# mathcom/G2Vec

Hardware: AMD Instinct MI355X
Metric: cbow_paths_per_sec (higher is better)
Workload: dtype fp32; 1 GPU; model=g2vec-cbow, global_batch=60057, seq_len=80, parallelism=dp1, hidden=128, num_repetition=10, num_repetition_global=10, hipgraph_active=True, grad_allreduce_bytes_per_epoch=30092, step_includes=full-batch fwd+bwd+allreduce+dense-Adam + post-update train/val ACC evals

## Files before the change

g2vec_amd/models/cbow.py:

```python
from __future__ import annotations

import dataclasses
import operator
import time
from typing import Any, List, Optional

import torch

from .. import ops
from ..config import G2VecConfig
from ..parallel.dist import DistContext, single
from ..paths import PathSet, subset


class _CpuEvent:
    def record(self):
        pass

    def synchronize(self):
        pass


@dataclasses.dataclass
class TrainResult:
    W_ih: torch.Tensor
    stop_epoch: int
    acc_val: float
    acc_tr: float
    epochs_run: int
    acc_val_history: List[float]
    epoch_times_s: List[float]
    wall_to_acc_s: Optional[float]


@dataclasses.dataclass
class TrainState:
    W: torch.Tensor
    who: torch.Tensor
    mW: torch.Tensor
    vW: torch.Tensor
    mO: torch.Tensor
    vO: torch.Tensor
    W_keep: torch.Tensor
    tr: PathSet
    vl: PathSet
    plan: Any
    inv_b: float
    batches: list
    W16: Optional[torch.Tensor] = None
    t_adam: int = 0
    epoch_idx: int = 0
    s_buf: Optional[torch.Tensor] = None
    lrt_buf: Optional[torch.Tensor] = None
    counts_buf: Optional[torch.Tensor] = None
    dO_buf: Optional[torch.Tensor] = None
    ev_genes: Optional[torch.Tensor] = None
    ev_offsets: Optional[torch.Tensor] = None
    ev_labels: Optional[torch.Tensor] = None
    graph: Any = None
    graph_failed: bool = False
    kbufs: Optional[tuple] = None
    kgraph: Any = None
    kblock_k: Optional[int] = None
    kgraph_failed: bool = False
    run_bufs: Optional[tuple] = None
    pipe_bufs: Optional[tuple] = None


EPOCH_TENSORS = ("W", "who", "mW", "vW", "mO", "vO", "dO_buf")
_epoch_tensors = operator.attrgetter(*EPOCH_TENSORS)


def accuracies(counts, n_tr: int, n_vl: int) -> tuple:
    return float(counts[0]) / max(n_tr, 1), float(counts[1]) / max(n_vl, 1)


def capture_graph(body, log, label: str):
    try:
        g = torch.cuda.CUDAGraph()
        with torch.cuda.graph(g, capture_error_mode="thread_local"):
            body()
        return g
    except Exception as e:
        log(label % repr(e))
        return None


class StopTracker:

    def __init__(self, early_stop: bool, before_val: float = -1.0,
                 before_tr: float = -1.0, hist: Optional[list] = None):
        self.early_stop = early_stop
        self.before_val, self.before_tr = before_val, before_tr
        self.hist: List[float] = hist if hist is not None else []
# ... 159 lines not shown

        use_general = cfg.trainer_path == "general"
        if cfg.batch_size == 0:
            tr = self._locality_sort(tr)
            vl = self._locality_sort(vl)
        plan = ops.build_scatter_plan(tr.genes, tr.offsets, self.G,
                                      slabs=not use_general)
        if self.n_tr_global + self.n_vl_global == 0:
            raise ValueError(
                "no paths to train on: the integrated path set is empty "
                "(every walk was dropped as a cross-group duplicate, or "
                "the PCC-thresholded graphs have no edges — check the "
                "expression signal / --pcc-threshold)")
        P_loc = tr.n_paths
        bs = cfg.batch_size if cfg.batch_size > 0 else max(P_loc, 1)
        st = TrainState(
            W=W, who=who, mW=torch.zeros_like(W), vW=torch.zeros_like(W),
            mO=torch.zeros_like(who), vO=torch.zeros_like(who),
            W_keep=W.clone(), tr=tr, vl=vl, plan=plan,
            inv_b=1.0 / max(self.n_tr_global, 1),
            batches=[(i, min(i + bs, P_loc)) for i in range(0, P_loc, bs)])
        if use_general and cfg.dtype != "fp32":
            st.W16 = (W.bfloat16() if cfg.dtype == "bf16" else W.half())
        if self.ctx.world > 1 and cfg.batch_size > 0:
            nb = torch.tensor([float(len(st.batches))], dtype=torch.float64,
                              device=self.device)
            self.ctx.allreduce_max_(nb)
            while len(st.batches) < int(nb.item()):
                st.batches.append((P_loc, P_loc))
        if not use_general:
            st.s_buf = torch.empty(self.G, dtype=torch.float32,
                                   device=self.device)
            ops.gemv_rows(W, who, st.s_buf)
        st.lrt_buf = torch.zeros(1, dtype=torch.float32, device=self.device)
        st.counts_buf = torch.zeros(2, dtype=torch.float32, device=self.device)
        if not use_general and tr.n_paths + vl.n_paths > 0:
            off_vl = vl.offsets.int() + tr.offsets[-1]
            st.ev_genes = torch.cat([tr.genes, vl.genes]).contiguous()
            st.ev_offsets = torch.cat([tr.offsets, off_vl[1:]]).contiguous()
            st.ev_labels = torch.cat([tr.labels, vl.labels]).contiguous()
        if not use_general and cfg.batch_size == 0:
            st.dO_buf = torch.zeros(tr.n_paths, dtype=torch.float32,
                                    device=self.device)
            if tr.n_paths > 0:
                _l, _c, d0 = ops.cbow_fwd_scalar(
                    st.s_buf, tr.genes, tr.offsets, tr.labels, st.inv_b, True)
                st.dO_buf.copy_(d0)
        return st

    def _epoch_body_fast(self, st, counts_out=None, lrt_slot=None,
                         reduce_counts: bool = True) -> None:
        cfg = self.cfg
        tr, vl = st.tr, st.vl
        if counts_out is None:
            counts_out = st.counts_buf
        if self.device.type != "cuda" or st.ev_genes is None:
            counts_out.zero_()
        if lrt_slot is not None:
            lrt = lrt_slot
        else:
            lrt = st.lrt_buf if self.device.type == "cuda" else None
        c = ops.scatter_dO(tr.genes, tr.offsets, st.dO_buf, self.G,
                           plan=st.plan)
        self.ctx.allreduce_(c)
        ops.adam_rank1_fused(st.W, st.mW, st.vW, c, st.who, st.mO, st.vO,
                             st.t_adam, cfg.lr, self.B1, self.B2, self.EPS,
                             lrt_buf=lrt)
        ops.gemv_rows(st.W, st.who, st.s_buf)
        if st.ev_genes is not None:
            ops.cbow_eval_counts_(st.s_buf, st.ev_genes, st.ev_offsets,
                                  st.ev_labels, tr.n_paths, counts_out,
                                  dO=st.dO_buf, inv_b=st.inv_b)
        if reduce_counts:
            self.ctx.allreduce_(counts_out)

    def run_epoch(self, st) -> tuple:
        cfg = self.cfg
        fast_full = cfg.trainer_path != "general" and cfg.batch_size == 0
        if fast_full:
            self._step_epoch(st)
            return self._accs(st.counts_buf.cpu().numpy())

        for (lo, hi) in st.batches:
            b_inv = (st.inv_b if cfg.batch_size == 0 else
                     (1.0 / ((hi - lo) * self.ctx.world) if hi > lo else 0.0))
            st.t_adam += 1
            if cfg.trainer_path == "general":
                self._step_general(st, lo, hi, b_inv, st.t_adam)
            else:
                self._step_fast(st, lo, hi, b_inv, st.t_adam)
        if cfg.trainer_path == "general":
            acc_tr = self._accuracy(st.W, st.W16, st.who, st.tr, self.n_tr_global)
            acc_val = self._accuracy(st.W, st.W16, st.who, st.vl, self.n_vl_global)
        else:
            ops.gemv_rows(st.W, st.who, st.s_buf)
            counts = torch.empty(2, dtype=torch.float32, device=self.device)
            for k, split in enumerate((st.tr, st.vl)):
                if split.n_paths == 0:
                    counts[k] = 0.0
                    continue
                _l, corr, _d = ops.cbow_fwd_scalar(
                    st.s_buf, split.genes, split.offsets, split.labels, 1.0, False)
                counts[k] = corr.sum()
            self.ctx.allreduce_(counts)
            acc_tr, acc_val = self._accs(counts.cpu().numpy())
# ... 26 lines not shown
                "    (hipGraph capture unavailable: %s; running eager)")
            st.graph_failed = st.graph is None

    def _launch_epoch(self, st, slot: int, pinned, snaps, events,
                      keep: bool = True) -> None:
        self._step_epoch(st)
        pinned[slot].copy_(st.counts_buf, non_blocking=True)
        if keep:
            snaps[slot][0].copy_(st.W)
            snaps[slot][1].copy_(st.who)
        events[slot].record()

    KBLOCK = 8

    def pick_kblock(self, n_epochs: int) -> int:
        n = max(int(n_epochs), 1)
        if n <= 64:
            return n
        for k in range(64, 1, -1):
            if n % k == 0:
                return k
        return self.KBLOCK

    def _ensure_kgraph(self, st, k: Optional[int] = None) -> None:
        if self.device.type != "cuda" or not self.cfg.use_hipgraph:
            return
        if not self.ctx.graph_capture_ok():
            return
        K = max(int(k), 1) if k is not None else (st.kblock_k or self.KBLOCK)
        if st.kbufs is None or st.kbufs[0].numel() != K:
            st.kbufs = (
                torch.empty(K, dtype=torch.float32, device=self.device),
                torch.zeros(K, 2, dtype=torch.float32, device=self.device))
            st.kgraph = None
        if st.kgraph is None and not st.kgraph_failed:
            klrt, kcounts = st.kbufs

            def bodies():
                for j in range(K):
                    self._epoch_body_fast(st, counts_out=kcounts[j],
                                          lrt_slot=klrt[j:j + 1],
                                          reduce_counts=False)
            st.kgraph = capture_graph(
                bodies, self.log, "    (k-epoch block graph unavailable: "
                                  "%s; running per-epoch)")
            if st.kgraph is not None:
                st.kblock_k = K
            else:
                st.kgraph_failed = True

    def kblock_eligible(self, st, n_epochs: int, early_stop: bool) -> bool:
        return (not early_stop and not st.kgraph_failed and
                st.ev_genes is not None and n_epochs >= 2)

    def _run_epochs_kblocked(self, st, n_epochs: int, on_epoch):
        on_gpu = self.device.type == "cuda"
        if st.epoch_idx == 0:
            warm = [self.run_epoch(st)]
        else:
            warm = []
        self._ensure_kgraph(st)
        n_rest = n_epochs - len(warm)
        K = st.kblock_k if st.kgraph is not None else None
        n_blocked = (n_rest // K) * K if K else 0
        sched_vals = torch.tensor(
            [ops.tf1_lr_t(self.cfg.lr, self.B1, self.B2, st.t_adam + i)
             for i in range(1, n_rest + 1)], dtype=torch.float32)
        if on_gpu:
            cap = max(n_rest, 1)
            if st.run_bufs is None or st.run_bufs[0].numel() < cap:
                st.run_bufs = (
                    torch.empty(cap, dtype=torch.float32, pin_memory=True),
                    torch.empty(cap, dtype=torch.float32,
                                device=self.device),
                    torch.zeros(cap, 2, dtype=torch.float32,
# ... 285 lines not shown
```

g2vec_amd/ops/__init__.py:

```python
from __future__ import annotations

from typing import NamedTuple, Optional

import torch

from . import cpu_ref

_NATIVE = None
_NATIVE_ERR: Optional[BaseException] = None
try:
    from g2vec_amd import _C as _NATIVE
except Exception as e:
    _NATIVE_ERR = e


def native_available() -> bool:
    return _NATIVE is not None


def native():
    if _NATIVE is None:
        raise RuntimeError(
            "g2vec_amd._C HIP extension is not importable on this host — the GPU "
            "compute path refuses to fall back to eager PyTorch. Build it in-tree "
            "with `python setup.py build_ext --inplace` (PYTORCH_ROCM_ARCH=gfx950). "
            f"Import error was: {_NATIVE_ERR!r}")
    return _NATIVE


def random_walks(row_ptr, col_idx, weights, sources, num_repetition: int,
                 len_path: int, seed: int):
    if row_ptr.is_cuda:
        return native().random_walks(row_ptr, col_idx, weights, sources,
                                     num_repetition, len_path, seed)
    return cpu_ref.random_walks(row_ptr, col_idx, weights, sources,
                                num_repetition, len_path, seed)


def cbow_fwd_scalar(s, genes, offsets, labels, inv_b: float, want_grad: bool):
    if s.is_cuda:
        loss, correct, dO = native().cbow_fwd_scalar(
            s, genes, offsets, labels, float(inv_b), bool(want_grad))
        return loss, correct, (dO if want_grad else None)
    return cpu_ref.cbow_fwd_scalar(s, genes, offsets, labels, inv_b, want_grad)


def cbow_eval_counts_(s, genes, offsets, labels, p_split: int,
                      counts: torch.Tensor, dO: Optional[torch.Tensor] = None,
                      inv_b: float = 1.0, scan=None) -> None:
    if s.is_cuda:
        if scan is not None:
            pathid, piece, cap = scan
            native().cbow_eval_scan_(s, genes, pathid, offsets, labels,
                                     int(p_split), int(cap), piece, counts,
                                     dO=dO, inv_b=float(inv_b))
            return
        native().cbow_eval_counts_(s, genes, offsets, labels, int(p_split),
                                   counts, dO=dO, inv_b=float(inv_b))
        return
    _l, corr, d = cpu_ref.cbow_fwd_scalar(s, genes, offsets, labels, inv_b,
                                          dO is not None)
    counts[0] += corr[:p_split].sum()
    counts[1] += corr[p_split:].sum()
    if dO is not None:
        dO.copy_(d[:p_split])


class ScatterPlan(NamedTuple):
    inst_path: torch.Tensor
    seg_start: torch.Tensor
    seg_gene: torch.Tensor
    slab_seg_ptr: Optional[list] = None


SLAB_BYTES = 3 << 20


def build_scatter_plan(genes: torch.Tensor, offsets: torch.Tensor,
                       n_genes: int, _force_slabs: bool = False,
                       slabs: bool = True) -> ScatterPlan:
    counts = (offsets[1:] - offsets[:-1]).long()
    P = len(counts)
    path_of = torch.repeat_interleave(
        torch.arange(P, device=genes.device), counts)
    slab_paths = SLAB_BYTES // 4
    n_slabs = ((P + slab_paths - 1) // slab_paths
               if slabs and (genes.is_cuda or _force_slabs) else 1)
    if n_slabs <= 1:
        sorted_key, perm = torch.sort(genes.long(), stable=True)
    else:
        key = (path_of // slab_paths) * n_genes + genes.long()
        sorted_key, perm = torch.sort(key, stable=True)
    inst_path = path_of[perm].int().contiguous()
    seg_key, seg_counts = torch.unique_consecutive(sorted_key,
                                                   return_counts=True)
    seg_start = torch.zeros(len(seg_key) + 1, dtype=torch.int64,
                            device=genes.device)
    torch.cumsum(seg_counts, 0, out=seg_start[1:])
    if n_slabs <= 1:
        return ScatterPlan(inst_path, seg_start.int().contiguous(),
                           seg_key.int().contiguous())
    seg_slab = seg_key // n_genes
    seg_gene = (seg_key - seg_slab * n_genes).int().contiguous()
    ptr = torch.searchsorted(
        seg_slab, torch.arange(n_slabs + 1, device=genes.device)).cpu()
    return ScatterPlan(inst_path, seg_start.int().contiguous(), seg_gene,
                       [int(x) for x in ptr])


def _plan_slabs(plan: ScatterPlan):
    ptr = plan.slab_seg_ptr
    if ptr is None:
        if plan.seg_gene.numel():
            yield plan.seg_start, plan.seg_gene
        return
    for a, b in zip(ptr[:-1], ptr[1:]):
        if b > a:
            yield plan.seg_start[a:b + 1], plan.seg_gene[a:b]


def scatter_dO(genes, offsets, dO, n_genes: int,
               plan: Optional[ScatterPlan] = None):
    if dO.is_cuda:
        if plan is None:
            plan = build_scatter_plan(genes, offsets, n_genes)
        c = torch.zeros(n_genes, dtype=torch.float32, device=dO.device)
        for seg_start, seg_gene in _plan_slabs(plan):
            native().scatter_dO_det_(plan.inst_path, seg_start, seg_gene,
                                     dO, c)
        return c
    return cpu_ref.scatter_dO(genes, offsets, dO, n_genes)


def trunc_normal_(out: torch.Tensor, std: float, seed: int) -> None:
    if out.is_cuda:
        native().trunc_normal_(out, float(std), int(seed))
        return
    cpu_ref.trunc_normal_(out, std, seed)


def tf1_lr_t(lr: float, b1: float, b2: float, t: int) -> float:
    return lr * (1.0 - b2 ** t) ** 0.5 / (1.0 - b1 ** t)


def _lrt_buf(lrt_buf, W, t: int, lr: float, b1: float, b2: float):
    if lrt_buf is not None:
        return lrt_buf
    return torch.tensor([tf1_lr_t(lr, b1, b2, t)], dtype=torch.float32,
                        device=W.device)


def adam_rank1(W, m, v, c, who, t: int, lr: float, b1: float, b2: float,
               eps: float, lrt_buf: Optional[torch.Tensor] = None) -> None:
    if W.is_cuda:
        lrt_buf = _lrt_buf(lrt_buf, W, t, lr, b1, b2)
        native().adam_rank1(W, m, v, c, who, lrt_buf, float(b1), float(b2),
                            float(eps))
        return
    cpu_ref.adam_rank1(W, m, v, c, who, t, lr, b1, b2, eps)


def adam_rank1_fused(W, m, v, c, who, mO, vO, t: int, lr: float,
                     b1: float, b2: float, eps: float,
# ... 18 lines not shown
    cpu_ref.adam_dense(W, m, v, grad, t, lr, b1, b2, eps)


def cbow_fwd(W, who, genes, offsets, labels, inv_b: float, want_grad: bool,
             act: int = 0):
    if W.is_cuda:
        loss, correct, dO, H = native().cbow_fwd(
            W, who, genes, offsets, labels, float(inv_b), bool(want_grad),
            act=int(act))
        if not want_grad:
            return loss, correct, None, None
        return loss, correct, dO, H
    return cpu_ref.cbow_fwd(W, who, genes, offsets, labels, inv_b, want_grad,
                            act=act)


def cbow_bwd_rows(who, genes, offsets, dO, n_genes: int,
                  plan: Optional[ScatterPlan] = None,
                  H_pre: Optional[torch.Tensor] = None):
    if dO.is_cuda:
        if plan is None:
            plan = build_scatter_plan(genes, offsets, n_genes, slabs=False)
        if plan.slab_seg_ptr is not None:
            raise RuntimeError(
                "cbow_bwd_rows needs a single-pass plan "
                "(build_scatter_plan(..., slabs=False)), got a slab-blocked one")
        return native().cbow_bwd_rows(who, plan.inst_path, plan.seg_start,
                                      plan.seg_gene, dO, int(n_genes),
                                      Hpre=H_pre)
    return cpu_ref.cbow_bwd_rows(who, genes, offsets, dO, n_genes,
                                 H_pre=H_pre)


def gemv_rows(W, x, out) -> None:
    if W.is_cuda:
        native().gemv_rows_(W, x, out)
        return
    torch.mv(W, x, out=out)


def gemv_cols(W, c, out) -> None:
    if W.is_cuda:
        native().gemv_cols_(W, c, out)
        return
    torch.mv(W.t(), c, out=out)


REP_MAX = 32


def _rep_R(t: torch.Tensor, name: str) -> int:
    if t.dim() != 2 or t.dtype != torch.float32 or not t.is_contiguous():
        raise ValueError(f"{name} must be a contiguous float32 [rows, R] tensor")
    R = int(t.shape[1])
    if not 1 <= R <= REP_MAX:
        raise ValueError(f"{name}: R must be in [1, {REP_MAX}], got {R}")
    return R


def cbow_eval_counts_rep_(s_R, genes, offsets, labels, p_split: int,
                          counts_R: torch.Tensor,
                          dO_R: Optional[torch.Tensor] = None,
                          inv_b: float = 1.0) -> None:
    R = _rep_R(s_R, "s_R")
    if s_R.is_cuda:
        native().cbow_eval_counts_rep_(s_R, genes, offsets, labels,
                                       int(p_split), counts_R, dO_R=dO_R,
                                       inv_b=float(inv_b))
        return
    for r in range(R):
        cnt = torch.zeros(2, dtype=torch.float32)
# ... 270 lines not shown
```

g2vec_amd/ops/csrc/bindings.hip:

```cpp
#include <torch/extension.h>
#include <c10/hip/HIPStream.h>
#include <hip/hip_runtime.h>

#include <climits>
#include <cstdio>
#include <functional>
#include <initializer_list>
#include <optional>
#include <cstring>
#include <fstream>
#include <sstream>
#include <string>
#include <type_traits>
#include <vector>

#include "g2vec_kernels.hip"

namespace {

inline void check_gpu_cont(const torch::Tensor& t, const char* name) {
  TORCH_CHECK(t.is_cuda(), name, " must be on the GPU");
  TORCH_CHECK(t.is_contiguous(), name, " must be contiguous");
}
inline void check_f32(const torch::Tensor& t, const char* name) {
// ... 157 lines not shown
inline void check_offs(const torch::Tensor& offs, long long P) {
  TORCH_CHECK(offs.numel() == P + 1, "offs must have P + 1 elements");
}
inline void check_p_split(long long p_split, long long P) {
  TORCH_CHECK(p_split >= 0 && p_split <= P, "p_split must be in [0, P]");
}
inline void check_seg_start(const torch::Tensor& seg_start, int n_seg) {
  TORCH_CHECK(seg_start.numel() == (long long)n_seg + 1,
              "seg_start must have n_seg + 1 elements");
}

std::vector<torch::Tensor> cbow_fwd_scalar(torch::Tensor s, torch::Tensor genes,
                                           torch::Tensor offs, torch::Tensor labels,
                                           double inv_b, bool want_grad) {
  CHECK_F32(s); CHECK_I32(genes); CHECK_I32(offs); CHECK_F32(labels);
  check_same_device(s, {genes, offs, labels});
  const long long P = labels.numel();
  check_offs(offs, P);
  auto loss = torch::empty({P}, opts_on(s));
  auto correct = torch::empty({P}, opts_on(s));
  auto dO = torch::empty({want_grad ? P : 0}, opts_on(s));
  if (P == 0) return {loss, correct, dO};
  launch(cbow_fwd_scalar_kernel, grid_for(P, 16, 2048), 0, f32(s), i32(genes),
         i32(offs), f32(labels), P, inv_b, f32(loss), f32(correct),
         want_grad ? f32(dO) : nullptr);
  return {loss, correct, dO};
}

void fold_partials(const torch::Tensor& partials, torch::Tensor& counts) {
  launch(fold_partials_kernel, 1, 0, f32(partials), partials.size(0),
         f32(counts));
}

void cbow_eval_counts_(torch::Tensor s, torch::Tensor genes, torch::Tensor offs,
                       torch::Tensor labels, int64_t p_split,
                       torch::Tensor counts,
                       std::optional<torch::Tensor> dO, double inv_b) {
  if (dO) {
    CHECK_F32(*dO);
    TORCH_CHECK(dO->numel() >= p_split,
                "dO must cover the train split (p < p_split)");
  }
  CHECK_F32(s); CHECK_I32(genes); CHECK_I32(offs); CHECK_F32(labels);
  CHECK_F32(counts);
  check_same_device(s, {genes, offs, labels, counts});
  if (dO) check_same_device(s, {*dO});
  TORCH_CHECK(counts.numel() == 2, "counts must have 2 elements");
  const long long P = labels.numel();
  check_offs(offs, P);
  check_p_split(p_split, P);
  if (P == 0) return;
  const long long G = s.numel();
  const char* lds_env = getenv("G2VEC_EVAL_LDS");
  const long long lds_cap = lds_env ? atoll(lds_env) : 0;
  const bool lds = G * 4 <= lds_cap && G * 4 <= 158 * 1024;
  const int grid =
      grid_for(P, 16, lds ? env_int_min1("G2VEC_EVAL_LDS_GRID", 1024)
                          : env_int_min1("G2VEC_EVAL_GRID", 2048));
  auto partials = torch::empty({grid, 2}, opts_on(s));
  if (lds) {
    launch(cbow_eval_counts_lds_kernel, grid, G * 4, f32(s), i32(genes),
           i32(offs), f32(labels), P, p_split, f32(partials), f32(dO), inv_b,
           G);
  } else {
    launch(cbow_eval_counts_kernel, grid, 0, f32(s), i32(genes), i32(offs),
           f32(labels), P, p_split, f32(partials), f32(dO), inv_b);
  }
  fold_partials(partials, counts);
}

void cbow_eval_scan_(torch::Tensor s, torch::Tensor genes,
                     torch::Tensor pathid, torch::Tensor offs,
                     torch::Tensor labels, int64_t p_split, int64_t cap,
                     torch::Tensor piece, torch::Tensor counts,
                     std::optional<torch::Tensor> dO, double inv_b) {
  CHECK_F32(s); CHECK_I32(genes); CHECK_I32(pathid); CHECK_I32(offs);
  CHECK_F32(labels); CHECK_F32(piece); CHECK_F32(counts);
  check_same_device(s, {genes, pathid, offs, labels, piece, counts});
  const long long P = labels.numel();
  const long long nnz = genes.numel();
  const int cap_i = int_arg(cap, "cap");
  check_offs(offs, P);
  check_p_split(p_split, P);
  TORCH_CHECK(pathid.numel() == nnz,
              "pathid must have one element per element of genes");
  TORCH_CHECK(piece.numel() >= P * cap, "piece buffer too small");
  if (dO) {
    CHECK_F32(*dO);
    check_same_device(s, {*dO});
    TORCH_CHECK(dO->numel() >= p_split, "dO must cover the train split");
  }
  if (P == 0) return;
  const long long G = s.numel();
  const bool lds = G * 4 <= 48 * 1024;
  launch(eval_scan_kernel, grid_for(nnz, 256, lds ? 1536 : GRID_MAX),
         lds ? G * sizeof(float) : 0, f32(s), i32(genes), i32(pathid),
         i32(offs), nnz, cap_i, f32(piece), lds ? G : 0);
  const int grid_b = grid_for(P, 256, 2048);
  auto partials = torch::empty({grid_b, 2}, opts_on(s));
  launch(eval_finish_kernel, grid_b, 0, f32(piece), i32(offs), f32(labels), P,
         p_split, cap_i, f32(partials), f32(dO), inv_b);
// ... 147 lines not shown
  launch(pcc_edges_kernel, grid_for(E, 4), 0, f32(zt), i32(edge_idx), E, S,
         1.0f / (float)n_group, f32(out));
  return out;
}

torch::Tensor corr_gemm(torch::Tensor zt, int64_t n_group) {
  CHECK_F32(zt);
  TORCH_CHECK(zt.dim() == 2, "zt must be [G, S]");
  check_gfx950("corr_gemm", "MFMA kernel (use pcc_mode=edge)");
  const int G = int_arg(zt.size(0), "zt.size(0)");
  const int S = int_arg(zt.size(1), "zt.size(1)");
  const long long ntile = ((long long)G + 63) / 64;
  TORCH_CHECK(ntile * ntile <= (long long)INT_MAX, "corr_gemm: zt.size(0) = ",
              G, " needs ", ntile * ntile,
              " tiles, over the 2^31 - 1 blocks of one launch "
              "(use pcc_mode=edge)");
  const int S4 = ((S + 3) / 4) * 4;
  const size_t lds = 2ull * 64 * S4 * sizeof(float);
  TORCH_CHECK(lds <= 160 * 1024,
              "corr_gemm: S too large for the LDS-staged tile (use pcc_mode=edge)");
  auto C = torch::empty({G, G}, opts_on(zt));
  launch(corr_gemm_kernel, (unsigned)(ntile * ntile), lds, f32(zt), f32(C), G,
         S, S4, 1.0f / (float)n_group);
  return C;
}

void trunc_normal_(torch::Tensor out, double std, int64_t seed) {
  CHECK_F32(out);
  const long long n = (long long)out.numel();
  if (n == 0) return;
  launch(trunc_normal_kernel, grid_for(n, 256), 0, f32(out), n, std, seed);
}

void gemv_rows_(torch::Tensor W, torch::Tensor x, torch::Tensor out) {
  CHECK_F32(W); CHECK_F32(x); CHECK_F32(out);
  check_same_device(W, {x, out});
  TORCH_CHECK(W.dim() == 2, "W must be [G, h]");
  const long long G = W.size(0);
  const int h = int_arg(W.size(1), "W.size(1)");
  const int hpl = hpl_for(h);
  TORCH_CHECK(out.numel() == G && x.numel() == h, "gemv_rows shape mismatch");
  dispatch_hpl(hpl, [&](auto HPL) {
    launch(gemv_rows_kernel<decltype(HPL)::value>, row_wave_grid(G), 0, f32(W),
           f32(x), G, h, f32(out));
  });
}

void gemv_cols_(torch::Tensor W, torch::Tensor c, torch::Tensor out) {
  CHECK_F32(W); CHECK_F32(c); CHECK_F32(out);
  check_same_device(W, {c, out});
  TORCH_CHECK(W.dim() == 2, "W must be [G, h]");
  const long long G = W.size(0);
  const int h = int_arg(W.size(1), "W.size(1)");
  const int cpt = (h >= 256) ? h / 256 : 1;
  TORCH_CHECK(h % 64 == 0 && cpt >= 1 && cpt <= 4 && (cpt & (cpt - 1)) == 0,
              "gemv_cols needs hidden 64*k with h/256 in {<=1,2,4}");
  TORCH_CHECK(out.numel() == h && c.numel() == G, "gemv_cols shape mismatch");
  const int grid = grid_for(G, 8, 2048);
  auto partials = torch::empty({grid, h}, opts_on(W));
  dispatch_cpt(cpt, [&](auto CPT) {
    launch(gemv_cols_kernel<decltype(CPT)::value>, grid, 0, f32(W), f32(c), G,
           h, f32(partials));
  });
  launch(fold_cols_kernel, (h + 3) / 4, 0, f32(partials), grid, h, f32(out));
}

inline int check_rep_table(const torch::Tensor& t, const char* name) {
  check_f32(t, name);
  TORCH_CHECK(t.dim() == 2, name, " must be [rows, R]");
  const long long R = t.size(1);
  TORCH_CHECK(R >= 1 && R <= REP_MAX, name, ": R must be in [1, ", REP_MAX,
              "], got ", R);
  TORCH_CHECK(t.numel() < (1LL << 31), name, " must have < 2^31 elements");
  return (int)R;
}

template <typename F>
// ... 470 lines not shown
      q = (*end == '\t') ? end + 1 : end;
    }
    while (*q == '\r' || *q == '\n') ++q;
    TORCH_CHECK(*q == '\0',
                path, ":", ln, ": gene '", genes.back(),
                "' has more than ", S, " values (one per sample column)");
  }
  TORCH_CHECK(!genes.empty(), path,
              ": no expression rows (empty or header-only file)");
  const size_t G = genes.size();
  auto t = torch::from_blob(vals.data(), {(long long)G, (long long)S},
                            torch::TensorOptions().dtype(at::kFloat))
               .clone();
  return {genes, samples, t.t().contiguous()};
}

}

PYBIND11_MODULE(TORCH_EXTENSION_NAME, m) {
  m.def("random_walks", &random_walks, "CSR biased random walks (gfx950)");
  m.def("cbow_fwd_scalar", &cbow_fwd_scalar, "scalar CBOW forward + loss");
  m.def("scatter_dO_det_", &scatter_dO_det_,
        "deterministic c += X^T dO (one slab, out-arg)");
  m.def("cbow_eval_scan_", &cbow_eval_scan_,
        py::arg("s"), py::arg("genes"), py::arg("pathid"), py::arg("offs"),
        py::arg("labels"), py::arg("p_split"), py::arg("cap"),
        py::arg("piece"), py::arg("counts"),
        py::arg("dO") = py::none(), py::arg("inv_b") = 1.0,
        "instance-parallel fused eval (segmented scan + finish)");
  m.def("cbow_eval_counts_", &cbow_eval_counts_,
        py::arg("s"), py::arg("genes"), py::arg("offs"), py::arg("labels"),
        py::arg("p_split"), py::arg("counts"),
        py::arg("dO") = py::none(), py::arg("inv_b") = 1.0,
        "fused train/val correct-count eval (in-place counts[2])");
  m.def("adam_rank1", &adam_rank1,
        py::arg("W"), py::arg("m"), py::arg("v"), py::arg("c"),
        py::arg("who"), py::arg("lrt"), py::arg("b1"), py::arg("b2"),
        py::arg("eps"), py::arg("mO") = py::none(), py::arg("vO") = py::none(),
        "TF1 Adam, rank-1 grad (mO/vO given: fused dW_ho + who update)");
  m.def("adam_dense", &adam_dense, "TF1 Adam, dense grad");
  m.def("cbow_fwd", &cbow_fwd,
        py::arg("W"), py::arg("who"), py::arg("genes"), py::arg("offs"),
        py::arg("labels"), py::arg("inv_b"), py::arg("want_grad"),
        py::arg("act") = 0,
        "row-gather CBOW forward (act: 0 linear, 1 ReLU)");
  m.def("cbow_bwd_rows", &cbow_bwd_rows,
        py::arg("who"), py::arg("inst_path"), py::arg("seg_start"),
        py::arg("seg_gene"), py::arg("dO"), py::arg("n_genes"),
        py::arg("Hpre") = py::none(),
        "deterministic scatter CBOW backward (Hpre = ReLU mask source)");
  m.def("pcc_edges", &pcc_edges, "per-edge |PCC|");
  m.def("corr_gemm", &corr_gemm, "MFMA f32 correlation GEMM");
  m.def("trunc_normal_", &trunc_normal_,
        "seeded +-2sigma truncated-normal fill (K9)");
  m.def("gemv_rows_", &gemv_rows_, "s = W @ x (wave-per-row GEMV, out-arg)");
  m.def("gemv_cols_", &gemv_cols_, "out = W^T c (partials + fold, out-arg)");
  m.def("cbow_eval_counts_rep_", &cbow_eval_counts_rep_,
        py::arg("s_R"), py::arg("genes"), py::arg("offs"), py::arg("labels"),
        py::arg("p_split"), py::arg("counts_R"),
        py::arg("dO_R") = py::none(), py::arg("inv_b") = 1.0,
        "replica-batched fused eval: counts_R [R, 2] + train dlogits dO_R");
  m.def("scatter_dO_rep_", &scatter_dO_rep_,
        "replica-batched deterministic c_R += X^T dO_R (accumulating)");
  m.def("adam_rank1_rep", &adam_rank1_rep,
        "replica-batched fused tail: rank-1 Adam + dW_ho fold + who Adam");
  m.def("gemv_rows_rep_", &gemv_rows_rep_,
        "s_R[:, r] = W[r] @ who[r] (replica-minor out-arg)");
  m.def("bf16_copy", &bf16_copy, "f32 -> bf16 cast kernel");
  m.def("kmeans_step", &kmeans_step,
        py::arg("X"), py::arg("C"), py::arg("prev"), py::arg("labels"),
        py::arg("C_new"), py::arg("sums"), py::arg("counts"),
        py::arg("n_changed"), py::arg("inertia"),
        "one fused Lloyd iteration (assign + sums/counts/inertia + C')");
  m.def("kmeans_mind2_", &kmeans_mind2_,
        "d2 = min(d2, |x - c|^2) for one new centre (k-means++)");
  m.def("row_norms_", &row_norms_, "row L2 norms, f64-accumulated (out-arg)");
  m.def("t_scores_", &t_scores_, "|pooled t| per gene column (out-arg)");
  m.def("col_moments_", &col_moments_,
        "f64 column sums of x and x*x (out-args)");
  m.def("perm_t_stats_", &perm_t_stats_,
        "t^2 per (relabelling, gene), MFMA f32 (out-arg)");
  m.def("perm_t_counts_", &perm_t_counts_,
        "per-gene exceed counts + per-relabelling max t^2 (out-args)");
  m.def("rank_columns_", &rank_columns_, py::arg("expr"), py::arg("ranks"),
        "average ranks per gene column, ties included (out-arg)");
  m.def("ranksum_scores_", &ranksum_scores_, py::arg("expr"),
        py::arg("labels"), py::arg("z"), py::arg("auc"),
        "rank-sum |z| and AUC per gene column (out-args)");
// ... 16 lines not shown
```

g2vec_amd/ops/csrc/g2vec_kernels.hip:

```cpp
#include <hip/hip_fp16.h>
#include <hip/hip_runtime.h>
#include <cstdint>

#ifdef G2VEC_DEBUG
#define G2V_ASSERT(cond) \
  do { if (!(cond)) __builtin_trap(); } while (0)
#else
#define G2V_ASSERT(cond) do { } while (0)
#endif

#define WAVE 64

__device__ __forceinline__ uint64_t sm64_next(uint64_t& s) {
  s += 0x9E3779B97F4A7C15ULL;
  uint64_t z = s;
  z = (z ^ (z >> 30)) * 0xBF58476D1CE4E5B9ULL;
  z = (z ^ (z >> 27)) * 0x94D049BB133111EBULL;
  return z ^ (z >> 31);
}

__device__ __forceinline__ double u01_from(uint64_t r) {
  return (double)(r >> 11) * (1.0 / 9007199254740992.0);
}

// ... 366 lines not shown
                        long long P, long long p_split,
                        float* __restrict__ partials,
                        float* __restrict__ dO, float inv_b) {
  eval_counts_body(s, genes, offs, labels, P, p_split, partials, dO, inv_b,
                   blockDim.x / SUBW);
}

extern "C" __global__ void __launch_bounds__(256)
cbow_eval_counts_lds_kernel(const float* __restrict__ s,
                            const int* __restrict__ genes,
                            const int* __restrict__ offs,
                            const float* __restrict__ labels,
                            long long P, long long p_split,
                            float* __restrict__ partials,
                            float* __restrict__ dO, float inv_b, int G) {
  extern __shared__ float s_lds[];
  for (int g = threadIdx.x; g < G; g += blockDim.x) s_lds[g] = s[g];
  __syncthreads();
  eval_counts_body(s_lds, genes, offs, labels, P, p_split, partials, dO,
                   inv_b, blockDim.x / SUBW);
}

extern "C" __global__ void __launch_bounds__(256)
fold_partials_kernel(const float* __restrict__ partials, int n_blocks,
                     float* __restrict__ counts) {
  float c0 = 0.f, c1 = 0.f;
  for (int b = threadIdx.x; b < n_blocks; b += blockDim.x) {
    c0 += partials[2 * b];
    c1 += partials[2 * b + 1];
  }
  block_fold2(c0, c1, counts);
}

#define REP_MAX 32
typedef float f32x4 __attribute__((ext_vector_type(4)));

template <bool VEC>
__device__ __forceinline__ f32x4 rep_gather4(const float* __restrict__ tab,
                                             int row, int R, int t) {
  if (VEC)
    return ((const f32x4*)tab)[(long long)row * (R >> 2) + t];
  const float* p = tab + (long long)row * R;
  f32x4 o;
#pragma unroll
  for (int k = 0; k < 4; ++k) {
    const int r = 4 * t + k;
    o[k] = p[r < R ? r : R - 1];
  }
  return o;
}

template <int NT, bool VEC>
__global__ void __launch_bounds__(256)
cbow_eval_counts_rep_kernel(const float* __restrict__ s_R,
                            const int* __restrict__ genes,
                            const int* __restrict__ offs,
                            const float* __restrict__ labels,
                            long long P, long long p_split, int R,
                            float* __restrict__ partials,
                            float* __restrict__ dO_R, float inv_b) {
  constexpr int NR = NT * 4;
  constexpr int NK = NR > SUBW ? 2 : 1;
  const int subs_per_block = blockDim.x / SUBW;
  const int sublane = threadIdx.x & (SUBW - 1);
  const int sub = threadIdx.x / SUBW;
  const long long stride = (long long)gridDim.x * subs_per_block;
// ... 53 lines not shown
    }
    p = pn; lo = lo_n; hi = hi_n; y = y_n;
  }
  __shared__ float sm[4 * 256];
#pragma unroll
  for (int k = 0; k < NK; ++k) {
    sm[(2 * k) * 256 + threadIdx.x] = c0[k];
    sm[(2 * k + 1) * 256 + threadIdx.x] = c1[k];
  }
  __syncthreads();
  if (threadIdx.x < 2 * NK * SUBW) {
    const int which = threadIdx.x / SUBW;
    const int r = sublane + (which >> 1) * SUBW;
    float tot = 0.f;
    for (int sb = 0; sb < subs_per_block; ++sb)
      tot += sm[which * 256 + sb * SUBW + sublane];
    if (r < R)
      partials[((long long)blockIdx.x * R + r) * 2 + (which & 1)] = tot;
  }
}

extern "C" __global__ void __launch_bounds__(256)
fold_partials_rep_kernel(const float* __restrict__ partials, int n_blocks,
                         int R, float* __restrict__ counts_R) {
  const int r = blockIdx.x;
  float c0 = 0.f, c1 = 0.f;
  for (int b = threadIdx.x; b < n_blocks; b += blockDim.x) {
    c0 += partials[((long long)b * R + r) * 2];
    c1 += partials[((long long)b * R + r) * 2 + 1];
  }
  block_fold2(c0, c1, counts_R + 2 * r);
}

extern "C" __global__ void __launch_bounds__(256)
scatter_do_det_kernel(const int* __restrict__ inst_path,
                      const int* __restrict__ seg_start,
                      const int* __restrict__ seg_gene, int n_seg,
                      const float* __restrict__ dO, float* __restrict__ c) {
  const int lane = threadIdx.x & (WAVE - 1);
  const int wib = threadIdx.x >> 6;
  const int wpb = blockDim.x >> 6;
  for (long long sidx = (long long)blockIdx.x * wpb + wib; sidx < n_seg;
       sidx += (long long)gridDim.x * wpb) {
    const int lo = seg_start[sidx], hi = seg_start[sidx + 1];
    float p0 = 0.f, p1 = 0.f, p2 = 0.f, p3 = 0.f;
    int i = lo + lane;
    for (; i + 3 * WAVE < hi; i += 4 * WAVE) {
      p0 += dO[inst_path[i]];
      p1 += dO[inst_path[i + WAVE]];
      p2 += dO[inst_path[i + 2 * WAVE]];
      p3 += dO[inst_path[i + 3 * WAVE]];
    }
    for (; i < hi; i += WAVE) p0 += dO[inst_path[i]];
    const float v = wave_sum((p0 + p1) + (p2 + p3));
    if (lane == 0) c[seg_gene[sidx]] += v;
  }
}

template <int NT, bool VEC>
__global__ void __launch_bounds__(256)
scatter_do_rep_kernel(const int* __restrict__ inst_path,
                      const int* __restrict__ seg_start,
                      const int* __restrict__ seg_gene, int n_seg,
                      const float* __restrict__ dO_R, int R,
                      float* __restrict__ c_R) {
  constexpr int NR = NT * 4;
  const int lane = threadIdx.x & (WAVE - 1);
  const int wib = threadIdx.x >> 6;
  const int wpb = blockDim.x >> 6;
  for (long long sidx = (long long)blockIdx.x * wpb + wib; sidx < n_seg;
       sidx += (long long)gridDim.x * wpb) {
    const int lo = seg_start[sidx], hi = seg_start[sidx + 1];
    float acc[4][NR];
#pragma unroll
    for (int q = 0; q < 4; ++q)
#pragma unroll
      for (int r = 0; r < NR; ++r) acc[q][r] = 0.f;
    int i = lo + lane;
    for (; i + 3 * WAVE < hi; i += 4 * WAVE) {
      int ip[4];
#pragma unroll
      for (int q = 0; q < 4; ++q) ip[q] = inst_path[i + q * WAVE];
#pragma unroll
      for (int t = 0; t < NT; ++t) {
        f32x4 d[4];
#pragma unroll
        for (int q = 0; q < 4; ++q) d[q] = rep_gather4<VEC>(dO_R, ip[q], R, t);
#pragma unroll
// ... 47 lines not shown
    f32x4 ww = __builtin_nontemporal_load(&W4[i]);
#pragma unroll
    for (int k = 0; k < 4; ++k) {
      if (gw_partials) gw_acc[k] += cg * ww[k];
      const float grad = cg * wj[k];
      mm[k] = b1 * mm[k] + (1.f - b1) * grad;
      vv[k] = b2 * vv[k] + (1.f - b2) * grad * grad;
      ww[k] -= lr_t * mm[k] / (sqrtf(vv[k]) + eps);
    }
    __builtin_nontemporal_store(mm, &m4[i]);
    __builtin_nontemporal_store(vv, &v4[i]);
    __builtin_nontemporal_store(ww, &W4[i]);
  }
  if (gw_partials) {
    __shared__ float gw_slots[256 * 4];
    float* slot = gw_slots + (lrow * h4 + j4) * 4;
#pragma unroll
    for (int k = 0; k < 4; ++k) slot[k] = gw_acc[k];
    __syncthreads();
    if (lrow == 0) {
      f32x4 tot = {0.f, 0.f, 0.f, 0.f};
      for (int r = 0; r < rpb; ++r) {
        const float* sl = gw_slots + (r * h4 + j4) * 4;
#pragma unroll
        for (int k = 0; k < 4; ++k) tot[k] += sl[k];
      }
      float* out = gw_partials + (long long)blockIdx.x * h + j4 * 4;
#pragma unroll
      for (int k = 0; k < 4; ++k) out[k] = tot[k];
    }
  }
}

extern "C" __global__ void __launch_bounds__(256)
fold_gw_adam_kernel(const float* __restrict__ partials, int n_blocks, int h,
                    float* __restrict__ who, float* __restrict__ mO,
                    float* __restrict__ vO,
                    const float* __restrict__ lr_t_ptr, float b1, float b2,
                    float eps) {
  const float lr_t = lr_t_ptr[0];
  const int lane = threadIdx.x & (WAVE - 1);
  const int wib = threadIdx.x >> 6;
  const int wpb = blockDim.x >> 6;
  for (int i = blockIdx.x * wpb + wib; i < h; i += gridDim.x * wpb) {
    float g = 0.f;
    for (int b = lane; b < n_blocks; b += WAVE)
      g += partials[(long long)b * h + i];
    g = wave_sum(g);
    if (lane == 0) {
      const float mm = b1 * mO[i] + (1.f - b1) * g;
      const float vv = b2 * vO[i] + (1.f - b2) * g * g;
      mO[i] = mm;
      vO[i] = vv;
      who[i] -= lr_t * mm / (sqrtf(vv) + eps);
    }
  }
}

extern "C" __global__ void __launch_bounds__(256)
adam_dense_kernel(float* __restrict__ W, float* __restrict__ m,
                  float* __restrict__ v, const float* __restrict__ grad,
                  long long n, const float* __restrict__ lr_t_ptr, float b1,
                  float b2, float eps) {
  const float lr_t = lr_t_ptr[0];
  for (long long i = (long long)blockIdx.x * blockDim.x + threadIdx.x; i < n;
       i += (long long)gridDim.x * blockDim.x) {
    const float g = grad[i];
    float mm = b1 * m[i] + (1.f - b1) * g;
    float vv = b2 * v[i] + (1.f - b2) * g * g;
    m[i] = mm; v[i] = vv;
    W[i] -= lr_t * mm / (sqrtf(vv) + eps);
  }
}

template <typename WT, int HPL>
__global__ void __launch_bounds__(256)
cbow_fwd_kernel(const WT* __restrict__ W, const float* __restrict__ who,
                const int* __restrict__ genes, const int* __restrict__ offs,
                const float* __restrict__ labels, long long P, float inv_b,
                int h, float* __restrict__ H, float* __restrict__ loss,
                float* __restrict__ correct, float* __restrict__ dO,
                int act) {
  const int lane = threadIdx.x & (WAVE - 1);
  const int wib = threadIdx.x >> 6;
  const int wpb = blockDim.x >> 6;
  const int col0 = lane * HPL;
  for (long long p = (long long)blockIdx.x * wpb + wib; p < P;
// ... 124 lines not shown
  const int kk = lane >> 4;
  for (int k0 = 0; k0 < S4; k0 += 4) {
    float av[2], bv[2];
#pragma unroll
    for (int a = 0; a < 2; ++a)
      av[a] = At[(wr * 32 + a * 16 + fr) * S4 + k0 + kk];
#pragma unroll
    for (int b = 0; b < 2; ++b)
      bv[b] = Bt[(wc * 32 + b * 16 + fr) * S4 + k0 + kk];
#pragma unroll
    for (int a = 0; a < 2; ++a)
#pragma unroll
      for (int b = 0; b < 2; ++b)
        acc[a][b] = __builtin_amdgcn_mfma_f32_16x16x4f32(av[a], bv[b],
                                                         acc[a][b], 0, 0, 0);
  }
#pragma unroll
  for (int a = 0; a < 2; ++a)
#pragma unroll
    for (int b = 0; b < 2; ++b)
#pragma unroll
      for (int reg = 0; reg < 4; ++reg) {
        const int ci = i0 + wr * 32 + a * 16 + (lane >> 4) * 4 + reg;
        const int cj = j0 + wc * 32 + b * 16 + (lane & 15);
        if (ci < G && cj < G)
          C[(long long)ci * G + cj] = acc[a][b][reg] * inv_s;
      }
#endif
}

template <int HPL>
__global__ void __launch_bounds__(256)
gemv_rows_kernel(const float* __restrict__ W, const float* __restrict__ x,
                 long long G, int h, float* __restrict__ out) {
  const int lane = threadIdx.x & (WAVE - 1);
  const int wib = threadIdx.x >> 6;
  const int wpb = blockDim.x >> 6;
  const int col0 = lane * HPL;
  float xv[HPL];
  __builtin_memcpy(xv, x + col0, HPL * sizeof(float));
  for (long long g = (long long)blockIdx.x * wpb + wib; g < G;
       g += (long long)gridDim.x * wpb) {
    float acc[HPL];
    __builtin_memcpy(acc, W + g * (long long)h + col0, HPL * sizeof(float));
    float p = 0.f;
#pragma unroll
    for (int k = 0; k < HPL; ++k) p += acc[k] * xv[k];
    const float o = wave_sum(p);
    if (lane == 0) out[g] = o;
  }
}


template <int CPT>
__global__ void __launch_bounds__(256)
gemv_cols_kernel(const float* __restrict__ W, const float* __restrict__ c,
                 long long G, int h, float* __restrict__ partials) {
  const int col0 = threadIdx.x * CPT;
  if (col0 >= h) return;
  float acc[CPT];
#pragma unroll
  for (int k = 0; k < CPT; ++k) acc[k] = 0.f;
  const long long rows_per_blk = (G + gridDim.x - 1) / gridDim.x;
  const long long lo = (long long)blockIdx.x * rows_per_blk;
  const long long hi = (lo + rows_per_blk < G) ? lo + rows_per_blk : G;
  for (long long g = lo; g < hi; ++g) {
    const float cg = c[g];
    float wv[CPT];
    __builtin_memcpy(wv, W + g * (long long)h + col0, CPT * sizeof(float));
#pragma unroll
    for (int k = 0; k < CPT; ++k) acc[k] += cg * wv[k];
  }
  float* p = partials + (long long)blockIdx.x * h + col0;
  __builtin_memcpy(p, acc, CPT * sizeof(float));
}

extern "C" __global__ void __launch_bounds__(256)
fold_cols_kernel(const float* __restrict__ partials, int n_blocks, int h,
                 float* __restrict__ out) {
  const int lane = threadIdx.x & (WAVE - 1);
  const int col = blockIdx.x * (blockDim.x >> 6) + (threadIdx.x >> 6);
  if (col >= h) return;
// ... 982 lines not shown
```

Before: 1.097 billion paths/s.

## Fuse buffer clears and partial folds across k-epoch graph; unroll scatter/fold loads

Reuses a persistent gradient buffer that the GEMV kernel zeroes as a side effect, removing a per-epoch memset and allocation. Inside the captured k-epoch graph, the eval kernels now write per-epoch partial tables and a single batched fold kernel reduces all K at the end, replacing K separate fold launches. The scatter and fold_gw_adam kernels unroll their gather loops with clamped indices so more loads are in flight at once. The cost is more code complexity and extra partial-table memory, plus some redundant clamped loads.

After: 1.241 billion paths/s (median of 6 runs). +13.2%, better.

```diff
diff --git a/g2vec_amd/models/cbow.py b/g2vec_amd/models/cbow.py
--- a/g2vec_amd/models/cbow.py
+++ b/g2vec_amd/models/cbow.py
@@ -51,6 +51,7 @@
     t_adam: int = 0
     epoch_idx: int = 0
     s_buf: Optional[torch.Tensor] = None
+    c_buf: Optional[torch.Tensor] = None
     lrt_buf: Optional[torch.Tensor] = None
     counts_buf: Optional[torch.Tensor] = None
     dO_buf: Optional[torch.Tensor] = None
@@ -60,6 +61,7 @@
     graph: Any = None
     graph_failed: bool = False
     kbufs: Optional[tuple] = None
+    kparts: Optional[torch.Tensor] = None
     kgraph: Any = None
     kblock_k: Optional[int] = None
     kgraph_failed: bool = False
@@ -285,6 +287,8 @@
             st.s_buf = torch.empty(self.G, dtype=torch.float32,
                                    device=self.device)
             ops.gemv_rows(W, who, st.s_buf)
+            st.c_buf = torch.zeros(self.G, dtype=torch.float32,
+                                   device=self.device)
         st.lrt_buf = torch.zeros(1, dtype=torch.float32, device=self.device)
         st.counts_buf = torch.zeros(2, dtype=torch.float32, device=self.device)
         if not use_general and tr.n_paths + vl.n_paths > 0:
@@ -302,9 +306,11 @@
         return st
 
     def _epoch_body_fast(self, st, counts_out=None, lrt_slot=None,
-                         reduce_counts: bool = True) -> None:
+                         reduce_counts: bool = True,
+                         partials_out=None) -> None:
         cfg = self.cfg
         tr, vl = st.tr, st.vl
+        on_gpu = self.device.type == "cuda"
         if counts_out is None:
             counts_out = st.counts_buf
         if self.device.type != "cuda" or st.ev_genes is None:
@@ -314,16 +320,18 @@
         else:
             lrt = st.lrt_buf if self.device.type == "cuda" else None
         c = ops.scatter_dO(tr.genes, tr.offsets, st.dO_buf, self.G,
-                           plan=st.plan)
+                           plan=st.plan, out=st.c_buf if on_gpu else None)
         self.ctx.allreduce_(c)
         ops.adam_rank1_fused(st.W, st.mW, st.vW, c, st.who, st.mO, st.vO,
                              st.t_adam, cfg.lr, self.B1, self.B2, self.EPS,
                              lrt_buf=lrt)
-        ops.gemv_rows(st.W, st.who, st.s_buf)
+        ops.gemv_rows(st.W, st.who, st.s_buf,
+                      clear=st.c_buf if on_gpu else None)
         if st.ev_genes is not None:
             ops.cbow_eval_counts_(st.s_buf, st.ev_genes, st.ev_offsets,
                                   st.ev_labels, tr.n_paths, counts_out,
-                                  dO=st.dO_buf, inv_b=st.inv_b)
+                                  dO=st.dO_buf, inv_b=st.inv_b,
+                                  partials=partials_out)
         if reduce_counts:
             self.ctx.allreduce_(counts_out)
 
@@ -416,15 +424,25 @@
             st.kbufs = (
                 torch.empty(K, dtype=torch.float32, device=self.device),
                 torch.zeros(K, 2, dtype=torch.float32, device=self.device))
+            st.kparts = None
             st.kgraph = None
         if st.kgraph is None and not st.kgraph_failed:
             klrt, kcounts = st.kbufs
+            if st.ev_genes is not None:
+                grid = ops.eval_grid(st.ev_labels.numel(), self.G)
+                if st.kparts is None or tuple(st.kparts.shape) != (K, grid, 2):
+                    st.kparts = torch.empty(K, grid, 2, dtype=torch.float32,
+                                            device=self.device)
+            kparts = st.kparts
 
             def bodies():
                 for j in range(K):
-                    self._epoch_body_fast(st, counts_out=kcounts[j],
-                                          lrt_slot=klrt[j:j + 1],
-                                          reduce_counts=False)
+                    self._epoch_body_fast(
+                        st, counts_out=kcounts[j], lrt_slot=klrt[j:j + 1],
+                        reduce_counts=False,
+                        partials_out=None if kparts is None else kparts[j])
+                if kparts is not None:
+                    ops.fold_partials_rows_(kparts, kcounts)
             st.kgraph = capture_graph(
                 bodies, self.log, "    (k-epoch block graph unavailable: "
                                   "%s; running per-epoch)")
diff --git a/g2vec_amd/ops/__init__.py b/g2vec_amd/ops/__init__.py
--- a/g2vec_amd/ops/__init__.py
+++ b/g2vec_amd/ops/__init__.py
@@ -47,7 +47,10 @@
 
 def cbow_eval_counts_(s, genes, offsets, labels, p_split: int,
                       counts: torch.Tensor, dO: Optional[torch.Tensor] = None,
-                      inv_b: float = 1.0, scan=None) -> None:
+                      inv_b: float = 1.0, scan=None,
+                      partials: Optional[torch.Tensor] = None) -> None:
+    if partials is not None and (not s.is_cuda or scan is not None):
+        raise ValueError("partials goes with the GPU subwave eval only")
     if s.is_cuda:
         if scan is not None:
             pathid, piece, cap = scan
@@ -56,7 +59,8 @@
                                      dO=dO, inv_b=float(inv_b))
             return
         native().cbow_eval_counts_(s, genes, offsets, labels, int(p_split),
-                                   counts, dO=dO, inv_b=float(inv_b))
+                                   counts, dO=dO, inv_b=float(inv_b),
+                                   partials=partials)
         return
     _l, corr, d = cpu_ref.cbow_fwd_scalar(s, genes, offsets, labels, inv_b,
                                           dO is not None)
@@ -64,6 +68,14 @@
     counts[1] += corr[p_split:].sum()
     if dO is not None:
         dO.copy_(d[:p_split])
+
+
+def eval_grid(P: int, G: int) -> int:
+    return int(native().eval_grid(int(P), int(G)))
+
+
+def fold_partials_rows_(partials: torch.Tensor, counts: torch.Tensor) -> None:
+    native().fold_partials_rows_(partials, counts)
 
 
 class ScatterPlan(NamedTuple):
@@ -120,15 +132,23 @@
 
 
 def scatter_dO(genes, offsets, dO, n_genes: int,
-               plan: Optional[ScatterPlan] = None):
+               plan: Optional[ScatterPlan] = None,
+               out: Optional[torch.Tensor] = None):
     if dO.is_cuda:
         if plan is None:
             plan = build_scatter_plan(genes, offsets, n_genes)
-        c = torch.zeros(n_genes, dtype=torch.float32, device=dO.device)
+        if out is None:
+            c = torch.zeros(n_genes, dtype=torch.float32, device=dO.device)
+        else:
+            if out.numel() != n_genes:
+                raise ValueError("out must have n_genes elements")
+            c = out
         for seg_start, seg_gene in _plan_slabs(plan):
             native().scatter_dO_det_(plan.inst_path, seg_start, seg_gene,
                                      dO, c)
         return c
+    if out is not None:
+        raise ValueError("out goes with the GPU path only")
     return cpu_ref.scatter_dO(genes, offsets, dO, n_genes)
 
 
@@ -213,11 +233,13 @@
                                  H_pre=H_pre)
 
 
-def gemv_rows(W, x, out) -> None:
-    if W.is_cuda:
-        native().gemv_rows_(W, x, out)
+def gemv_rows(W, x, out, clear: Optional[torch.Tensor] = None) -> None:
+    if W.is_cuda:
+        native().gemv_rows_(W, x, out, clear=clear)
         return
     torch.mv(W, x, out=out)
+    if clear is not None:
+        clear.zero_()
 
 
 def gemv_cols(W, c, out) -> None:
diff --git a/g2vec_amd/ops/csrc/bindings.hip b/g2vec_amd/ops/csrc/bindings.hip
--- a/g2vec_amd/ops/csrc/bindings.hip
+++ b/g2vec_amd/ops/csrc/bindings.hip
@@ -213,10 +213,38 @@
          f32(counts));
 }
 
+void fold_partials_rows_(torch::Tensor partials, torch::Tensor counts) {
+  CHECK_F32(partials); CHECK_F32(counts);
+  check_same_device(partials, {counts});
+  TORCH_CHECK(partials.dim() == 3 && partials.size(2) == 2,
+              "partials must be [K, grid, 2]");
+  const int K = int_arg(partials.size(0), "partials.size(0)");
+  const int grid = int_arg(partials.size(1), "partials.size(1)");
+  TORCH_CHECK(counts.dim() == 2 && counts.size(0) == K && counts.size(1) == 2,
+              "counts must be [K, 2]");
+  if (K == 0) return;
+  launch(fold_partials_rows_kernel, K, 0, f32(partials), grid, f32(counts));
+}
+
+struct EvalGeom { bool lds; int grid; };
+inline EvalGeom eval_geom(long long P, long long G) {
+  const char* lds_env = getenv("G2VEC_EVAL_LDS");
+  const long long lds_cap = lds_env ? atoll(lds_env) : 0;
+  const bool lds = G * 4 <= lds_cap && G * 4 <= 158 * 1024;
+  return {lds, grid_for(P, 16, lds ? env_int_min1("G2VEC_EVAL_LDS_GRID", 1024)
+                                   : env_int_min1("G2VEC_EVAL_GRID", 2048))};
+}
+
+int64_t eval_grid(int64_t P, int64_t G) {
+  TORCH_CHECK(P >= 0 && G >= 0, "eval_grid: P and G must be >= 0");
+  return eval_geom(P, G).grid;
+}
+
 void cbow_eval_counts_(torch::Tensor s, torch::Tensor genes, torch::Tensor offs,
                        torch::Tensor labels, int64_t p_split,
                        torch::Tensor counts,
-                       std::optional<torch::Tensor> dO, double inv_b) {
+                       std::optional<torch::Tensor> dO, double inv_b,
+                       std::optional<torch::Tensor> partials_out) {
   if (dO) {
     CHECK_F32(*dO);
     TORCH_CHECK(dO->numel() >= p_split,
@@ -230,15 +258,18 @@
   const long long P = labels.numel();
   check_offs(offs, P);
   check_p_split(p_split, P);
+  const long long G = s.numel();
+  const auto [lds, grid] = eval_geom(P, G);
+  if (partials_out) {
+    CHECK_F32(*partials_out);
+    check_same_device(s, {*partials_out});
+    TORCH_CHECK(partials_out->dim() == 2 && partials_out->size(0) == grid &&
+                    partials_out->size(1) == 2,
+                "partials must be [eval_grid(P, G), 2] = [", grid, ", 2]");
+  }
   if (P == 0) return;
-  const long long G = s.numel();
-  const char* lds_env = getenv("G2VEC_EVAL_LDS");
-  const long long lds_cap = lds_env ? atoll(lds_env) : 0;
-  const bool lds = G * 4 <= lds_cap && G * 4 <= 158 * 1024;
-  const int grid =
-      grid_for(P, 16, lds ? env_int_min1("G2VEC_EVAL_LDS_GRID", 1024)
-                          : env_int_min1("G2VEC_EVAL_GRID", 2048));
-  auto partials = torch::empty({grid, 2}, opts_on(s));
+  auto partials =
+      partials_out ? *partials_out : torch::empty({grid, 2}, opts_on(s));
   if (lds) {
     launch(cbow_eval_counts_lds_kernel, grid, G * 4, f32(s), i32(genes),
            i32(offs), f32(labels), P, p_split, f32(partials), f32(dO), inv_b,
@@ -247,7 +278,7 @@
     launch(cbow_eval_counts_kernel, grid, 0, f32(s), i32(genes), i32(offs),
            f32(labels), P, p_split, f32(partials), f32(dO), inv_b);
   }
-  fold_partials(partials, counts);
+  if (!partials_out) fold_partials(partials, counts);
 }
 
 void cbow_eval_scan_(torch::Tensor s, torch::Tensor genes,
@@ -461,7 +492,8 @@
   launch(trunc_normal_kernel, grid_for(n, 256), 0, f32(out), n, std, seed);
 }
 
-void gemv_rows_(torch::Tensor W, torch::Tensor x, torch::Tensor out) {
+void gemv_rows_(torch::Tensor W, torch::Tensor x, torch::Tensor out,
+                std::optional<torch::Tensor> clear) {
   CHECK_F32(W); CHECK_F32(x); CHECK_F32(out);
   check_same_device(W, {x, out});
   TORCH_CHECK(W.dim() == 2, "W must be [G, h]");
@@ -469,9 +501,15 @@
   const int h = int_arg(W.size(1), "W.size(1)");
   const int hpl = hpl_for(h);
   TORCH_CHECK(out.numel() == G && x.numel() == h, "gemv_rows shape mismatch");
+  if (clear) {
+    CHECK_F32(*clear);
+    check_same_device(W, {*clear});
+    TORCH_CHECK(clear->numel() == G, "clear must have one element per W row");
+    TORCH_CHECK(clear->data_ptr() != out.data_ptr(), "clear must not be out");
+  }
   dispatch_hpl(hpl, [&](auto HPL) {
     launch(gemv_rows_kernel<decltype(HPL)::value>, row_wave_grid(G), 0, f32(W),
-           f32(x), G, h, f32(out));
+           f32(x), G, h, f32(out), f32(clear));
   });
 }
 
@@ -1008,7 +1046,14 @@
         py::arg("s"), py::arg("genes"), py::arg("offs"), py::arg("labels"),
         py::arg("p_split"), py::arg("counts"),
         py::arg("dO") = py::none(), py::arg("inv_b") = 1.0,
-        "fused train/val correct-count eval (in-place counts[2])");
+        py::arg("partials") = py::none(),
+        "fused train/val correct-count eval (in-place counts[2]; partials "
+        "[eval_grid, 2] given: written instead, no fold)");
+  m.def("eval_grid", &eval_grid, py::arg("P"), py::arg("G"),
+        "block count of cbow_eval_counts_ = rows of its partial table");
+  m.def("fold_partials_rows_", &fold_partials_rows_, py::arg("partials"),
+        py::arg("counts"),
+        "counts [K, 2] = fold of K evals' partial tables [K, grid, 2]");
   m.def("adam_rank1", &adam_rank1,
         py::arg("W"), py::arg("m"), py::arg("v"), py::arg("c"),
         py::arg("who"), py::arg("lrt"), py::arg("b1"), py::arg("b2"),
@@ -1029,7 +1074,9 @@
   m.def("corr_gemm", &corr_gemm, "MFMA f32 correlation GEMM");
   m.def("trunc_normal_", &trunc_normal_,
         "seeded +-2sigma truncated-normal fill (K9)");
-  m.def("gemv_rows_", &gemv_rows_, "s = W @ x (wave-per-row GEMV, out-arg)");
+  m.def("gemv_rows_", &gemv_rows_, py::arg("W"), py::arg("x"), py::arg("out"),
+        py::arg("clear") = py::none(),
+        "s = W @ x (wave-per-row GEMV, out-arg; clear [G] given: zeroed too)");
   m.def("gemv_cols_", &gemv_cols_, "out = W^T c (partials + fold, out-arg)");
   m.def("cbow_eval_counts_rep_", &cbow_eval_counts_rep_,
         py::arg("s_R"), py::arg("genes"), py::arg("offs"), py::arg("labels"),
diff --git a/g2vec_amd/ops/csrc/g2vec_kernels.hip b/g2vec_amd/ops/csrc/g2vec_kernels.hip
--- a/g2vec_amd/ops/csrc/g2vec_kernels.hip
+++ b/g2vec_amd/ops/csrc/g2vec_kernels.hip
@@ -422,6 +422,18 @@
   block_fold2(c0, c1, counts);
 }
 
+extern "C" __global__ void __launch_bounds__(256)
+fold_partials_rows_kernel(const float* __restrict__ partials, int n_blocks,
+                          float* __restrict__ counts) {
+  partials += (long long)blockIdx.x * n_blocks * 2;
+  float c0 = 0.f, c1 = 0.f;
+  for (int b = threadIdx.x; b < n_blocks; b += blockDim.x) {
+    c0 += partials[2 * b];
+    c1 += partials[2 * b + 1];
+  }
+  block_fold2(c0, c1, counts + 2 * blockIdx.x);
+}
+
 #define REP_MAX 32
 typedef float f32x4 __attribute__((ext_vector_type(4)));
 
@@ -541,6 +553,11 @@
   block_fold2(c0, c1, counts_R + 2 * r);
 }
 
+#ifndef SCAT_U
+#define SCAT_U 8
+#endif
+static_assert(SCAT_U >= 4 && SCAT_U % 4 == 0, "SCAT_U: whole groups of 4");
+
 extern "C" __global__ void __launch_bounds__(256)
 scatter_do_det_kernel(const int* __restrict__ inst_path,
                       const int* __restrict__ seg_start,
@@ -552,17 +569,33 @@
   for (long long sidx = (long long)blockIdx.x * wpb + wib; sidx < n_seg;
        sidx += (long long)gridDim.x * wpb) {
     const int lo = seg_start[sidx], hi = seg_start[sidx + 1];
+    const int gene = seg_gene[sidx];
+    const float c_old = c[gene];
     float p0 = 0.f, p1 = 0.f, p2 = 0.f, p3 = 0.f;
-    int i = lo + lane;
-    for (; i + 3 * WAVE < hi; i += 4 * WAVE) {
-      p0 += dO[inst_path[i]];
-      p1 += dO[inst_path[i + WAVE]];
-      p2 += dO[inst_path[i + 2 * WAVE]];
-      p3 += dO[inst_path[i + 3 * WAVE]];
-    }
-    for (; i < hi; i += WAVE) p0 += dO[inst_path[i]];
+    int i0 = lo + lane;
+    for (int rem = hi - i0; rem + lane > 0;
+         rem -= SCAT_U * WAVE, i0 += SCAT_U * WAVE) {
+      int ip[SCAT_U];
+      float d[SCAT_U];
+#pragma unroll
+      for (int u = 0; u < SCAT_U; ++u)
+        ip[u] = inst_path[i0 + (u * WAVE < rem ? u * WAVE : rem - 1)];
+#pragma unroll
+      for (int u = 0; u < SCAT_U; ++u) d[u] = dO[ip[u]];
+#pragma unroll
+      for (int q = 0; q < SCAT_U / 4; ++q) {
+        const int k = 4 * q * WAVE;
+        const bool full = k + 3 * WAVE < rem;
+        p0 = (k < rem) ? p0 + d[4 * q] : p0;
+        p1 = full ? p1 + d[4 * q + 1] : p1;
+        p0 = (!full && k + WAVE < rem) ? p0 + d[4 * q + 1] : p0;
+        p2 = full ? p2 + d[4 * q + 2] : p2;
+        p0 = (!full && k + 2 * WAVE < rem) ? p0 + d[4 * q + 2] : p0;
+        p3 = full ? p3 + d[4 * q + 3] : p3;
+      }
+    }
     const float v = wave_sum((p0 + p1) + (p2 + p3));
-    if (lane == 0) c[seg_gene[sidx]] += v;
+    if (lane == 0) c[gene] = c_old + v;
   }
 }
 
@@ -676,6 +709,8 @@
   }
 }
 
+#define FOLD_U 16
+
 extern "C" __global__ void __launch_bounds__(256)
 fold_gw_adam_kernel(const float* __restrict__ partials, int n_blocks, int h,
                     float* __restrict__ who, float* __restrict__ mO,
@@ -687,16 +722,26 @@
   const int wib = threadIdx.x >> 6;
   const int wpb = blockDim.x >> 6;
   for (int i = blockIdx.x * wpb + wib; i < h; i += gridDim.x * wpb) {
+    const float mO_i = mO[i], vO_i = vO[i], who_i = who[i];
     float g = 0.f;
-    for (int b = lane; b < n_blocks; b += WAVE)
-      g += partials[(long long)b * h + i];
+    for (int b0 = lane; b0 - lane < n_blocks; b0 += FOLD_U * WAVE) {
+      float pv[FOLD_U];
+#pragma unroll
+      for (int u = 0; u < FOLD_U; ++u) {
+        const int b = b0 + u * WAVE;
+        pv[u] = partials[(long long)(b < n_blocks ? b : n_blocks - 1) * h + i];
+      }
+#pragma unroll
+      for (int u = 0; u < FOLD_U; ++u)
+        g = (b0 + u * WAVE < n_blocks) ? g + pv[u] : g;
+    }
     g = wave_sum(g);
     if (lane == 0) {
-      const float mm = b1 * mO[i] + (1.f - b1) * g;
-      const float vv = b2 * vO[i] + (1.f - b2) * g * g;
+      const float mm = b1 * mO_i + (1.f - b1) * g;
+      const float vv = b2 * vO_i + (1.f - b2) * g * g;
       mO[i] = mm;
       vO[i] = vv;
-      who[i] -= lr_t * mm / (sqrtf(vv) + eps);
+      who[i] = who_i - lr_t * mm / (sqrtf(vv) + eps);
     }
   }
 }
@@ -887,7 +932,8 @@
 template <int HPL>
 __global__ void __launch_bounds__(256)
 gemv_rows_kernel(const float* __restrict__ W, const float* __restrict__ x,
-                 long long G, int h, float* __restrict__ out) {
+                 long long G, int h, float* __restrict__ out,
+                 float* __restrict__ clear) {
   const int lane = threadIdx.x & (WAVE - 1);
   const int wib = threadIdx.x >> 6;
   const int wpb = blockDim.x >> 6;
@@ -902,7 +948,10 @@
 #pragma unroll
     for (int k = 0; k < HPL; ++k) p += acc[k] * xv[k];
     const float o = wave_sum(p);
-    if (lane == 0) out[g] = o;
+    if (lane == 0) {
+      out[g] = o;
+      if (clear) clear[g] = 0.0f;
+    }
   }
 }
 
```
